# Coloquinte/sleekit

Measured on AMD Instinct MI355X. Metric: Mweights/sec quantized (GPTQ 3-bit, 4096x4096 layer), higher is better.
Workload: dtype f64

## Files before the change

### sleekit_amd/csrc/api.hip

```cpp
#include "mfma32.h"
#include "mfma64.h"

namespace slk {

__global__ __launch_bounds__(256) void k_probe_f64(double *sink, int iters) {
    double4_t c0 = {0, 0, 0, 0}, c1 = c0, c2 = c0, c3 = c0;
    const double a = 1.0 + threadIdx.x * 1e-3, b = 1.0 - threadIdx.x * 1e-3;
    for (int i = 0; i < iters; ++i) {
        c0 = __builtin_amdgcn_mfma_f64_16x16x4f64(a, b, c0, 0, 0, 0);
        c1 = __builtin_amdgcn_mfma_f64_16x16x4f64(b, a, c1, 0, 0, 0);
        c2 = __builtin_amdgcn_mfma_f64_16x16x4f64(a, a, c2, 0, 0, 0);
        c3 = __builtin_amdgcn_mfma_f64_16x16x4f64(b, b, c3, 0, 0, 0);
    }
    const double4_t s = c0 + c1 + c2 + c3;
    if (s[0] + s[1] + s[2] + s[3] == 12345.678) sink[0] = s[0];
}

template <int NACC>
__global__ __launch_bounds__(256) void k_probe_f64_n(double *sink, int iters) {
    double4_t c[NACC];
    double a[NACC], b[NACC];
#pragma unroll
    for (int i = 0; i < NACC; ++i) {
        c[i] = (double4_t){0, 0, 0, 0};
// ... 67 lines not shown
}

using namespace slk;

extern "C" {

int slk_probe_chain(double *out, int iters, int mode, slk_stream_t stream) {
    SLK_REQUIRE(out && iters > 0, "bad arguments");
    hipStream_t s = as_stream(stream);
    SLK_RUN("probe_chain", 0, 0, s, k_probe_chain<<<1, 64, 0, s>>>(out, iters, mode));
    return SLK_OK;
}

size_t slk_workspace_bytes(int R, int n) {
    if (R < 0 || n <= 0) return 0;
    const size_t ld = (size_t)slk_factor_ld(n);
    const size_t rn = (size_t)(R > 0 ? R : 1) * (size_t)n;
    size_t factor = 2 * ld * ld * sizeof(double) + 2 * (ld / 64) * sizeof(int);
    size_t loop = 2 * rn * sizeof(float) + (size_t)n * sizeof(int) + 64 * sizeof(float) + 5 * 256;
    size_t search = rn * sizeof(float) + (size_t)(R + n) * sizeof(float) + (size_t)R * ((n + 127) / 128) * sizeof(float) + 4096;
    size_t error = 6 * (rn + 128 * (size_t)n) + 6 * (size_t)n * n + 4 * (size_t)R * ((n + 127) / 128) * sizeof(float) + 8192;
    size_t prep = 64 * sizeof(float) + (size_t)n * (sizeof(double) + 1);
    search += error;
    size_t m = factor;
    if (loop > m) m = loop;
    if (search > m) m = search;
    if (error > m) m = error;
    if (prep > m) m = prep;
    return m + (1u << 16);
}

size_t slk_workspace_bytes_batch(int batch, int rows_per_layer, int n) {
    if (batch < 1 || batch > 64 || rows_per_layer < 0 || n <= 0 || (long long)batch * rows_per_layer > 0x7fffffffLL) return 0;
    return slk_workspace_bytes(batch * rows_per_layer, n) + (size_t)(batch - 1) * 6 * (size_t)n * n +
           (size_t)batch * n * (sizeof(int) + sizeof(float)) + (size_t)(batch - 1) * 64 * sizeof(float) +
           4096;
}

int slk_probe_mfma_f64(double *sink, int blocks, int iters, slk_stream_t stream) {
    SLK_REQUIRE(sink && blocks > 0 && iters > 0, "bad arguments");
    hipStream_t s = as_stream(stream);
    SLK_RUN("probe_mfma_f64", 4.0 * 2048 * 4 * iters * blocks, 0, s, k_probe_f64<<<blocks, 256, 0, s>>>(sink, iters));
    return SLK_OK;
}

int slk_probe_mfma_f64_acc(double *sink, int blocks, int iters, int nacc, slk_stream_t stream) {
    SLK_REQUIRE(sink && blocks > 0 && iters > 0 && (nacc == 1 || nacc == 2 || nacc == 4 || nacc == 8 || nacc == 16), "bad arguments");
    hipStream_t s = as_stream(stream);
    if (nacc == 1)
        SLK_RUN("probe_mfma_f64", 1.0 * 2048 * 4 * iters * blocks, 0, s, k_probe_f64_n<1><<<blocks, 256, 0, s>>>(sink, iters));
    else if (nacc == 2)
        SLK_RUN("probe_mfma_f64", 2.0 * 2048 * 4 * iters * blocks, 0, s, k_probe_f64_n<2><<<blocks, 256, 0, s>>>(sink, iters));
    else if (nacc == 4)
        SLK_RUN("probe_mfma_f64", 4.0 * 2048 * 4 * iters * blocks, 0, s, k_probe_f64_n<4><<<blocks, 256, 0, s>>>(sink, iters));
    else if (nacc == 8)
        SLK_RUN("probe_mfma_f64", 8.0 * 2048 * 4 * iters * blocks, 0, s, k_probe_f64_n<8><<<blocks, 256, 0, s>>>(sink, iters));
    else
        SLK_RUN("probe_mfma_f64", 16.0 * 2048 * 4 * iters * blocks, 0, s, k_probe_f64_n<16><<<blocks, 256, 0, s>>>(sink, iters));
    return SLK_OK;
}

int slk_probe_mfma_f32(float *sink, int blocks, int iters, slk_stream_t stream) {
    SLK_REQUIRE(sink && blocks > 0 && iters > 0, "bad arguments");
    hipStream_t s = as_stream(stream);
    SLK_RUN("probe_mfma_f32", 4.0 * 4096 * 4 * iters * blocks, 0, s, k_probe_f32<<<blocks, 256, 0, s>>>(sink, iters));
    return SLK_OK;
}

}

#include <atomic>
#include <map>
#include <mutex>
#include <string>
#include <vector>
#include <strings.h>

namespace slk {
namespace {
const char *const kOptNames[OPT_COUNT] = {
    "NO_FAST_LEAF", "NO_DEFER", "NO_WINDOW2", "WIN_DBG", "NO_REGULAR_SEARCH", "NO_FAST_SEARCH_DIV",
    "NO_ERROR_SPLITK", "ERROR_CB", "NO_SYM_ERROR", "NO_BF16_ERROR", "NO_BF16_DMA", "NO_BF16_HESSIAN",
    "ERROR_F32_BELOW", "NO_BF16_ASYM", "NO_SYM_AVERAGE", "NO_WAVE_SEARCH", "LOOKAHEAD", "WINDOW_ROWS", "PANEL_SPLIT", "ROWS_BELOW_WIDE",
    "NO_LOOP_ERROR",
};
std::atomic<int> g_opts[OPT_COUNT];
std::once_flag g_opts_once;
void opts_from_env() {
    for (int i = 0; i < OPT_COUNT; ++i) {
        const std::string name = std::string("SLK_") + kOptNames[i];
        const char *v = getenv(name.c_str());
        int val = 0;
        if (v) {
            val = atoi(v);
            if (val == 0 && v[0] != '0') val = 1;
        }
        g_opts[i].store(val, std::memory_order_relaxed);
    }
}
int opt_index(const char *name) {
    if (!name) return -1;
    if (strncasecmp(name, "SLK_", 4) == 0) name += 4;
    for (int i = 0; i < OPT_COUNT; ++i)
        if (strcasecmp(name, kOptNames[i]) == 0) return i;
    return -1;
}
std::mutex g_lds_mu;
std::map<std::pair<const void *, int>, size_t> g_lds_set;
}

int opt(Opt o) {
    std::call_once(g_opts_once, opts_from_env);
    return g_opts[o].load(std::memory_order_relaxed);
}

namespace {
std::mutex g_helper_mu;
struct HelperRec {
    Helper h;
    int made;
};
std::map<std::pair<int, hipStream_t>, HelperRec> g_helpers;
}

hipError_t helper_for(hipStream_t main, int need, Helper *out) {
    if (need > HELPER_EVENTS) return hipErrorInvalidValue;
    int device = 0;
    hipError_t e = hipGetDevice(&device);
    if (e != hipSuccess) return e;
    std::lock_guard<std::mutex> lock(g_helper_mu);
    auto it = g_helpers.find({device, main});
    if (it == g_helpers.end()) {
        HelperRec r{};
        e = hipStreamCreateWithFlags(&r.h.stream, hipStreamNonBlocking);
        if (e != hipSuccess) return e;
        e = hipStreamCreateWithFlags(&r.h.stream2, hipStreamNonBlocking);
        if (e != hipSuccess) {
            (void)hipStreamDestroy(r.h.stream);
            return e;
        }
        r.h.events = new hipEvent_t[HELPER_EVENTS]();
        r.made = 0;
        it = g_helpers.emplace(std::make_pair(device, main), r).first;
    }
    HelperRec &r = it->second;
    const int had = r.made;
    while (r.made < need) {
        e = hipEventCreateWithFlags(&r.h.events[r.made], hipEventDisableTiming);
        if (e != hipSuccess) {
            while (r.made > had) (void)hipEventDestroy(r.h.events[--r.made]);
            if (had == 0) {
                (void)hipStreamDestroy(r.h.stream);
                (void)hipStreamDestroy(r.h.stream2);
                delete[] r.h.events;
                g_helpers.erase(it);
            }
            return e;
        }
        ++r.made;
    }
    *out = r.h;
    return hipSuccess;
}

static hipError_t release_helpers() {
    std::lock_guard<std::mutex> lock(g_helper_mu);
    hipError_t first = hipSuccess;
// ... 156 lines not shown
```

### sleekit_amd/csrc/common.h

```cpp
#pragma once

#include <hip/hip_runtime.h>
#include <stddef.h>
#include <stdint.h>
#include <stdio.h>

#include "../../include/sleekit_amd.h"

namespace slk {

void set_error(const char *fmt, ...);

#define SLK_REQUIRE(cond, ...)          \
    do {                                \
        if (!(cond)) {                  \
            slk::set_error(__VA_ARGS__); \
            return SLK_E_ARG;           \
        }                               \
    } while (0)

#define SLK_HIP(call)                                                                  \
    do {                                                                               \
        hipError_t e_ = (call);                                                        \
        if (e_ != hipSuccess) {                                                        \
            slk::set_error("%s failed: %s (%s:%d)", #call, hipGetErrorString(e_), __FILE__, __LINE__); \
            return SLK_E_HIP;                                                          \
        }                                                                              \
    } while (0)

#define SLK_LAUNCH_CHECK() SLK_HIP(hipGetLastError())

struct ProfScope {
    int slot;
    hipStream_t stream;
    ProfScope(const char *name, double flops, double bytes, hipStream_t s);
    ~ProfScope();
};

void prof_next_width(long workgroups);

#define SLK_RUN(name, flops, bytes, stream, ...)                 \
    do {                                                         \
        {                                                        \
            slk::ProfScope prof_scope_(name, flops, bytes, stream); \
            __VA_ARGS__;                                         \
        }                                                        \
        SLK_LAUNCH_CHECK();                                      \
    } while (0)

#define SLK_RUN_W(name, flops, bytes, wgs, stream, ...) \
    do {                                                \
        slk::prof_next_width((long)(wgs));              \
        SLK_RUN(name, flops, bytes, stream, __VA_ARGS__); \
    } while (0)

enum Opt {
    OPT_NO_FAST_LEAF,
    OPT_NO_DEFER,
    OPT_NO_WINDOW2,
    OPT_WIN_DBG,
    OPT_NO_REGULAR_SEARCH,
    OPT_NO_FAST_SEARCH_DIV,
    OPT_NO_ERROR_SPLITK,
    OPT_ERROR_CB,
    OPT_NO_SYM_ERROR,
    OPT_NO_BF16_ERROR,
    OPT_NO_BF16_DMA,
    OPT_NO_BF16_HESSIAN,
    OPT_ERROR_F32_BELOW,
    OPT_NO_BF16_ASYM,
    OPT_NO_SYM_AVERAGE,
    OPT_NO_WAVE_SEARCH,
    OPT_LOOKAHEAD,
    OPT_WINDOW_ROWS,
    OPT_PANEL_SPLIT,
    OPT_ROWS_BELOW_WIDE,
    OPT_NO_LOOP_ERROR,
    OPT_COUNT
};
int opt(Opt o);

struct Helper {
    hipStream_t stream;
    hipStream_t stream2;
    hipEvent_t *events;
};
constexpr int HELPER_EVENTS = 512;
hipError_t helper_for(hipStream_t main, int need, Helper *out);

hipError_t lds_opt_in(const void *kernel, size_t bytes);
#define SLK_LDS_OPT_IN(kernel, bytes) SLK_HIP(slk::lds_opt_in(reinterpret_cast<const void *>(kernel), (bytes)))

struct PtrTable {
    const float *p[64];
};

int row_errors_products(const float *W, const float *Q, const float *const *Hs, int batch, int rpl, int n, const int *sym_known,
                        float *row_err, float *G, void *workspace, size_t ws_bytes, slk_stream_t stream);

int loop_error_means(const float *const *Hs, int batch, int n, float *out, hipStream_t s);

static inline hipStream_t as_stream(slk_stream_t s) { return reinterpret_cast<hipStream_t>(s); }

static inline size_t align_up(size_t x, size_t a) { return (x + a - 1) / a * a; }

struct Arena {
    char *base;
    size_t size, used;
    Arena(void *p, size_t bytes) : base(static_cast<char *>(p)), size(bytes), used(0) {}
    template <class T>
    T *take(size_t count) {
        size_t off = align_up(used, 256);
        size_t end = off + count * sizeof(T);
        if (end > size || base == nullptr) return nullptr;
        used = end;
        return reinterpret_cast<T *>(base + off);
    }
};

struct Grid {
    float zero, step, top;
    const float *table;
    int n;
};

static inline Grid make_grid(int levels, double lo, double hi, const float *table = nullptr) {
    Grid g;
    g.zero = (float)lo;
    g.step = (float)((hi - lo) / (double)(levels - 1));
    g.top = (float)(levels - 1);
    g.table = table;
    g.n = levels;
    return g;
}

__device__ __forceinline__ float grid_pos(float x, const Grid g, float shift, float first, float last) {
    float t = (x - g.zero) / g.step;
    t = t + shift;
    t = rintf(t);
    return fminf(fmaxf(t, first), last);
}
__device__ __forceinline__ float grid_val(float t, const Grid g) { return t * g.step + g.zero; }
__device__ __forceinline__ float grid_value(float x, const Grid g) {
    return grid_val(grid_pos(x, g, 0.0f, 0.0f, g.top), g);
}

__device__ __forceinline__ int table_index(float x, const Grid g) {
    const float *lim = g.table + g.n;
    int lo = 0, hi = g.n - 1;
    while (lo < hi) {
        const int mid = (lo + hi) >> 1;
        if (lim[mid] <= x) lo = mid + 1; else hi = mid;
    }
    return lo;
}
__device__ __forceinline__ float cb_value(float x, const Grid g) { return g.table ? g.table[table_index(x, g)] : grid_value(x, g); }
__device__ __forceinline__ int cb_index(float x, const Grid g) {
    return g.table ? table_index(x, g) : (int)grid_pos(x, g, 0.0f, 0.0f, g.top);
}
__device__ __forceinline__ float cb_up(float x, const Grid g) {
// ... 95 lines not shown
```

### sleekit_amd/csrc/factor.hip

```cpp
#include <stdlib.h>

#include "mfma64.h"

namespace slk {

constexpr int PANEL = 64;
constexpr int OUTER_SMALL = 256, OUTER_LARGE = 512;
constexpr int LOOKAHEAD_MIN_TILES = 24;

__device__ long long g_panel_cycles[16];

constexpr int TP = 66;

struct PanelSmem {
    double t[PANEL][TP];
    double x[PANEL][TP];
    double a21[PANEL][TP];
    double lb[PANEL][TP];
    double rdiag[PANEL];
    int early_count;
};

#ifndef NEWTON_STEPS
#define NEWTON_STEPS 2
// ... 775 lines not shown
        const double *p = A + (size_t)(rows0 + (lane >> 4)) * ld + K0 + PANEL * q + 16 * wave + (lane & 15);
        return (double4_t){p[0], p[(size_t)4 * ld], p[(size_t)8 * ld], p[(size_t)12 * ld]};
    };
    TileRegs nx;
    tile_fetch<0>(nx, gx, tile_elem(0, 0), ld);
    double4_t c = load_c(0), cnext = load_c(nb > 1 ? 1 : 0);
    for (int q = 0; q < nb; ++q) {
        for (int s = 0; s <= q; ++s) {
            const bool tri = s == q;
            __syncthreads();
            tile_stash(sm.bt, nx);
            if (tri) blk_store_d(&sm.c[0][16 * wave], lane, c);
            __syncthreads();
            if (!tri) {
                if (s + 1 < q) tile_fetch<0>(nx, ga, tile_elem(q, s + 1), ld);
                else tile_fetch<0>(nx, gx, tile_elem(q, q), ld);
            } else if (q + 1 < nb) {
                tile_fetch<0>(nx, ga, tile_elem(q + 1, 0), ld);
            }
            if (!tri) {
                double4_t acc = {0.0, 0.0, 0.0, 0.0};
#pragma unroll
                for (int kq = 0; kq < 4; ++kq) acc = blk_mma_abt(&sm.own[s][0][16 * kq], &sm.bt[16 * wave][16 * kq], acc, 1.0, lane);
                c = c - acc;
            } else {
                double4_t acc = {0.0, 0.0, 0.0, 0.0};
#pragma unroll
                for (int k = 0; k < 4; ++k)
                    if (k <= wave) acc = blk_mma_abt(&sm.c[0][16 * k], &sm.bt[16 * wave][16 * k], acc, 1.0, lane);
#pragma unroll
                for (int j = 0; j < 4; ++j) A[(size_t)(rows0 + (lane >> 4) + 4 * j) * ld + K0 + PANEL * q + 16 * wave + (lane & 15)] = acc[j];
                blk_store_d(&sm.own[q][0][16 * wave], lane, acc);
                c = cnext;
                if (q + 2 < nb) cnext = load_c(q + 2);
            }
        }
    }
}

__global__ __launch_bounds__(256) void k_syrk_tiles(double *__restrict__ A, int ld, int ti0, int tj0, int ka,
                                                    int kb) {
    __shared__ __attribute__((aligned(16))) Tile64Smem sm;
    A += (size_t)blockIdx.z * ld * ld;
    const int bi = ti0 + blockIdx.y, bj = tj0 + blockIdx.x;
    if (bj > bi) return;
    Acc64 acc;
    acc.zero();
    const int t = threadIdx.x;
    const double *pa = A + ((size_t)bi * TILE + (t >> 2)) * ld + (t & 3) * 8;
    const double *pb = A + ((size_t)bj * TILE + (t >> 2)) * ld + (t & 3) * 8;
    double *pc = A + (size_t)bi * TILE * ld + (size_t)bj * TILE;
    Acc64 old;
    tile64_map(old, [&](int r, int c) { return pc[(size_t)r * ld + c]; });
    tile64_mac<false>(
        acc, sm, ka, kb, [&](int k0, double(&v)[8]) { load8d<true>(pa + k0, v); },
        [&](int k0, double(&v)[8]) { load8d<true>(pb + k0, v); });
    tile64_foreach2(old, acc, [&](int r, int c, double o, double v) { pc[(size_t)r * ld + c] = o - v; });
}

__global__ __launch_bounds__(256) void k_syrk_triangle(double *__restrict__ A, int ld, int t0, int m, int ka, int kb) {
    __shared__ __attribute__((aligned(16))) Tile64Smem sm;
    A += (size_t)blockIdx.z * ld * ld;
    const int total = m * (m + 1) / 2, per_xcd = (total + 7) / 8;
    const int lin = (blockIdx.x & 7) * per_xcd + (blockIdx.x >> 3);
    if (lin >= total) return;
    int row = (int)((sqrtf(8.0f * (float)lin + 1.0f) - 1.0f) * 0.5f);
    while (row * (row + 1) / 2 > lin) --row;
    while ((row + 1) * (row + 2) / 2 <= lin) ++row;
    const int bi = t0 + row, bj = t0 + lin - row * (row + 1) / 2;
    Acc64 acc;
    acc.zero();
    const int t = threadIdx.x;
    const double *pa = A + ((size_t)bi * TILE + (t >> 2)) * ld + (t & 3) * 8;
    const double *pb = A + ((size_t)bj * TILE + (t >> 2)) * ld + (t & 3) * 8;
    tile64_mac<false>(
        acc, sm, ka, kb, [&](int k0, double(&v)[8]) { load8d<true>(pa + k0, v); },
        [&](int k0, double(&v)[8]) { load8d<true>(pb + k0, v); });
    double *pc = A + (size_t)bi * TILE * ld + (size_t)bj * TILE;
    Acc64 old;
    tile64_map(old, [&](int r, int c) { return pc[(size_t)r * ld + c]; });
    tile64_foreach2(old, acc, [&](int r, int c, double o, double v) { pc[(size_t)r * ld + c] = o - v; });
}

template <int STAGE>
__global__ __launch_bounds__(256) void k_trtri_level(const double *__restrict__ L, double *__restrict__ X,
                                                     double *__restrict__ S, int ld, int nt, int s, int node0) {
    __shared__ __attribute__((aligned(16))) Tile64Smem sm;
    L += (size_t)blockIdx.z * ld * ld;
    X += (size_t)blockIdx.z * ld * ld;
    S += (size_t)blockIdx.z * ld * ld;
    const int id = blockIdx.x;
    const int per_node = s * s, node = node0 + id / per_node, in_node = id % per_node;
    const int deep = in_node / s, other = in_node % s;
    const int lo = node * 2 * s, mid = lo + s;
    const int bi = (STAGE == 0) ? mid + other : mid + (s - 1 - deep);
    const int bj = (STAGE == 0) ? lo + deep : lo + other;
    if (bi >= nt) return;
    Acc64 acc;
    acc.zero();
    const int t = threadIdx.x;
    if (STAGE == 0) {
        const double *pa = L + ((size_t)bi * TILE + (t >> 2)) * ld + (t & 3) * 8;
        const double *pb = X + (size_t)(t >> 3) * ld + (size_t)bj * TILE + (t & 7) * 2;
        tile64_mac<true>(
            acc, sm, bj * TILE, mid * TILE, [&](int k0, double(&v)[8]) { load8d<true>(pa + k0, v); },
            [&](int k0, double(&v)[8]) { load8d_cols(pb + (size_t)k0 * ld, v); });
        double *pc = S + (size_t)bi * TILE * ld + (size_t)bj * TILE;
        tile64_foreach(acc, [&](int r, int c, double v) { pc[(size_t)r * ld + c] = v; });
    } else {
        const double *pa = X + ((size_t)bi * TILE + (t >> 2)) * ld + (t & 3) * 8;
        const double *pb = S + (size_t)(t >> 3) * ld + (size_t)bj * TILE + (t & 7) * 2;
        tile64_mac<true>(
            acc, sm, mid * TILE, (bi + 1) * TILE, [&](int k0, double(&v)[8]) { load8d<true>(pa + k0, v); },
            [&](int k0, double(&v)[8]) { load8d_cols(pb + (size_t)k0 * ld, v); });
        double *pc = X + (size_t)bi * TILE * ld + (size_t)bj * TILE;
        tile64_foreach(acc, [&](int r, int c, double v) { pc[(size_t)r * ld + c] = -v; });
    }
}

__global__ __launch_bounds__(256) void k_flip_out(const double *__restrict__ X, int ld, int n,
                                                  double *__restrict__ U) {
    X += (size_t)blockIdx.z * ld * ld;
    U += (size_t)blockIdx.z * n * n;
    for (int i = blockIdx.x; i < n; i += gridDim.x) {
        const double *src = X + (size_t)(n - 1 - i) * ld;
        double *dst = U + (size_t)i * n;
        for (int j = threadIdx.x; j < n; j += blockDim.x) dst[j] = (j >= i) ? src[n - 1 - j] : 0.0;
    }
}

__global__ void k_clear_info(int *info, int *flags, int per_matrix) {
    if (threadIdx.x == 0) info[blockIdx.x] = 0;
    if (flags)
        for (int i = threadIdx.x; i < per_matrix; i += blockDim.x) flags[(size_t)blockIdx.x * per_matrix + i] = 0;
}

}

using namespace slk;

static int chol_inverse_impl(double *A, int batch, int n, double *U, int *info, void *workspace, size_t ws_bytes,
                             slk_stream_t stream, bool want_lookahead) {
    const int ld = slk_factor_ld(n);
    const int nt = ld / TILE;
    const unsigned B = (unsigned)batch;
    const double Bd = (double)batch;
    Arena ws(workspace, ws_bytes);
    double *X = ws.take<double>((size_t)ld * ld * batch);
    double *S = ws.take<double>((size_t)ld * ld * batch);
    int *flags = ws.take<int>((size_t)batch * 2 * nt);
    if (!X || !S || !flags) {
        set_error("workspace too small for %d factorisation(s) of %d x %d", batch, n, n);
        return SLK_E_WS;
    }
    hipStream_t s = as_stream(stream);
    const int OUTER = n >= 4096 ? OUTER_LARGE : OUTER_SMALL;
    SLK_LDS_OPT_IN(k_chol_panel, sizeof(PanelSmem));
    SLK_RUN_W("clear_info", 0, 4, 1, s, k_clear_info<<<B, 64, 0, s>>>(info, flags, 2 * nt));

    Helper helper{};
    const bool lookahead = (want_lookahead || opt(OPT_LOOKAHEAD)) && nt >= LOOKAHEAD_MIN_TILES + OUTER / TILE && nt / (OUTER / TILE) < HELPER_EVENTS / 3;
    if (lookahead) SLK_HIP(helper_for(s, 3 * (nt / (OUTER / TILE) + 1), &helper));
    const int sp = opt(OPT_PANEL_SPLIT);
    const bool chain = (sp == 0 || sp == 3) && slk_chain_addressable(ld);
    const bool split = !chain && !want_lookahead && sp != 2 && (sp == 1 || batch > 1 || n >= 8192);
    if (split) SLK_LDS_OPT_IN(k_panel_below, sizeof(BelowSmem));
    if (chain) {
        SLK_LDS_OPT_IN(k_chol_chain<false>, sizeof(PanelSmem));
        SLK_LDS_OPT_IN(k_chol_chain<true>, sizeof(PanelSmem));
        SLK_LDS_OPT_IN(k_chol_rows_below, sizeof(RowsBelowSmem));
    }
    int inv_done[2][16] = {{0}, {0}};
    auto inverse_nodes = [&](int tiles_done, hipStream_t st) -> int {
        int li = 0;
        for (int lvl = 1; lvl < nt; lvl *= 2, ++li) {
            const int all = (nt + 2 * lvl - 1) / (2 * lvl);
            for (int stage = 0; stage < 2; ++stage) {
                int ready;
                if (tiles_done >= nt) ready = all;
                else if (stage == 0) ready = tiles_done >= lvl ? (tiles_done - lvl) / (2 * lvl) + 1 : 0;
                else ready = tiles_done / (2 * lvl);
                if (ready > all) ready = all;
                const int first = inv_done[stage][li], count = ready - first;
                if (count <= 0) continue;
                inv_done[stage][li] = ready;
                double fl = 0, tiles = 0;
                for (int nd = first; nd < ready; ++nd) {
                    const int lo = nd * 2 * lvl, mid = lo + lvl, hi = lo + 2 * lvl < nt ? lo + 2 * lvl : nt;
                    for (int bi = mid; bi < hi; ++bi)
                        for (int bj = lo; bj < mid; ++bj) {
                            fl += 2.0 * 64 * 64 * 64 * (stage == 0 ? mid - bj : bi + 1 - mid);
                            tiles += 1;
                        }
                }
                if (tiles == 0) continue;
                dim3 grid(count * lvl * lvl, 1, B);
                if (stage == 0)
                    SLK_RUN_W("trtri_stage0", Bd * fl, Bd * (fl / 64 * 8.0 / 2 + tiles * 8.0 * 64 * 64), tiles * batch, st,
                              k_trtri_level<0><<<grid, 256, 0, st>>>(A, X, S, ld, nt, lvl, first));
                else
                    SLK_RUN_W("trtri_stage1", Bd * fl, Bd * (fl / 64 * 8.0 / 2 + tiles * 8.0 * 64 * 64), tiles * batch, st,
                              k_trtri_level<1><<<grid, 256, 0, st>>>(A, X, S, ld, nt, lvl, first));
            }
        }
        return SLK_OK;
    };
    const int EV = chain ? 3 : 2;
    int block = 0, forked = -1;
    int inverse_on_helper = -1;
    for (int K0 = 0; K0 < ld; K0 += OUTER) {
        const int K1 = K0 + OUTER < ld ? K0 + OUTER : ld;
        if (chain) {
            const int nb = (K1 - K0) / PANEL, below_tiles = (ld - K1) / PANEL;
            const double e = 64.0 * nb;
            SLK_RUN_W("chol_chain", Bd * e * e * e / 3.0, Bd * 12.0 * e * e, nb * batch, s,
                      k_chol_chain<false><<<dim3(nb, 1, B), 256, sizeof(PanelSmem), s>>>(A, ld, K0, nb, X, info, flags, opt(OPT_WIN_DBG) & 8));
            if (below_tiles > 0 && forked >= 0) {
                SLK_HIP(hipStreamWaitEvent(s, helper.events[EV * forked + 1], 0));
                forked = -1;
            }
            const int rw = opt(OPT_ROWS_BELOW_WIDE);
            const bool wide = rw == 1 || (rw == 0 && 4 * below_tiles * batch >= 1024);
            if (below_tiles > 0 && wide)
                SLK_RUN_W("chol_rows_below", Bd * 64.0 * below_tiles * e * e, Bd * (16.0 * 64 * below_tiles * e + 4.0 * e * e), below_tiles * batch, s,
                          k_chol_chain<true><<<dim3(below_tiles, 1, B), 256, sizeof(PanelSmem), s>>>(A, ld, K0, nb, X, info, flags, 0));
            else if (below_tiles > 0)
                SLK_RUN_W("chol_rows_below", Bd * 64.0 * below_tiles * e * e, Bd * (16.0 * 64 * below_tiles * e + 4.0 * e * e), 4 * below_tiles * batch, s,
                          k_chol_rows_below<<<dim3(4 * below_tiles, 1, B), 256, sizeof(RowsBelowSmem), s>>>(A, ld, K0, nb, X));
        }
        for (int k0 = K0; k0 < K1 && !chain; k0 += PANEL) {
            const int below = (ld - k0) / PANEL;
            const int kprev = k0 > K0 ? k0 - PANEL : -1;
            const int rest_cols = kprev >= 0 ? (K1 - k0) / PANEL - 1 : 0;
            int rest = 0;
            for (int c = 0; c < rest_cols; ++c) rest += nt - (k0 / TILE + 1 + c);
            const double prologue = kprev >= 0 ? (double)below * 2.0 * 64 * 64 * 64 + (double)below * 2.0 * 64 * 64 * 64 : 0.0;
            if (split) {
                const double pro1 = kprev >= 0 ? 2.0 * 64 * 64 * 64 : 0.0;
                SLK_RUN_W("chol_panel", Bd * (2.0 / 3.0 * 64 * 64 * 64 + pro1), Bd * 16.0 * 64 * 64, batch, s,
                          k_chol_panel<<<dim3(1, 1, B), 256, sizeof(PanelSmem), s>>>(A, ld, k0, kprev, 1, 0, X, info, opt(OPT_WIN_DBG) & 8));
                if (below - 1 + rest > 0) {
                    const int per_wg = 2;
                    const int nbw = (below - 1 + per_wg - 1) / per_wg;
                    SLK_RUN_W("chol_panel_below",
                              Bd * ((double)(below - 1) * 64 * 64 * 64 + (kprev >= 0 ? (double)(below - 1) * 2.0 * 64 * 64 * 64 : 0.0) +
                                    (double)rest * 2.0 * 64 * 64 * PANEL),
                              Bd * (24.0 * (below - 1) * 64 * 64 + (double)rest * 16.0 * 64 * 64), (nbw + rest) * batch, s,
                              k_panel_below<<<dim3(nbw + rest, 1, B), 256, sizeof(BelowSmem), s>>>(A, ld, k0, kprev, nbw, rest_cols, X, below - 1,
                                                                                                  per_wg));
                }
            } else {
                SLK_RUN_W("chol_panel",
                          Bd * (2.0 / 3.0 * 64 * 64 * 64 + (double)(below - 1) * 64 * 64 * 64 + prologue + (double)rest * 2.0 * 64 * 64 * PANEL),
                          Bd * (16.0 * below * 64 * 64 + (double)rest * 16.0 * 64 * 64), (below + rest) * batch, s,
                          k_chol_panel<<<dim3(below + rest, 1, B), 256, sizeof(PanelSmem), s>>>(A, ld, k0, kprev, below, rest_cols, X, info,
                                                                                                opt(OPT_WIN_DBG) & 8));
            }
        }
        const int t0 = K1 / TILE;
        if (nt > t0) {
            const int m = nt - t0, total = m * (m + 1) / 2;
            const double tiles = total;
            const int ahead = OUTER / TILE;
            if (lookahead && chain && m >= LOOKAHEAD_MIN_TILES) {
                SLK_HIP(hipEventRecord(helper.events[EV * block], s));
                const int nbn = ahead < m ? ahead : m, td = nbn * (nbn + 1) / 2;
                SLK_RUN_W("chol_syrk_ahead", Bd * td * 2.0 * 64 * 64 * (K1 - K0), Bd * (16.0 * nbn * 64 * (K1 - K0) + td * 16.0 * 64 * 64), td * batch, s,
                          k_syrk_tiles<<<dim3(nbn, nbn, B), 256, 0, s>>>(A, ld, t0, t0, K0, K1));
                SLK_HIP(hipStreamWaitEvent(helper.stream, helper.events[EV * block], 0));
                const int m2 = m - nbn, total2 = m2 * (m2 + 1) / 2;
                if (m2 > 0) {
                    SLK_RUN_W("chol_syrk_outer", Bd * (double)nbn * m2 * 2.0 * 64 * 64 * (K1 - K0), Bd * (8.0 * (ld - K1) * (K1 - K0) + (double)nbn * m2 * 16.0 * 64 * 64),
                              (double)nbn * m2 * batch, helper.stream,
                              k_syrk_tiles<<<dim3(nbn, m2, B), 256, 0, helper.stream>>>(A, ld, t0 + nbn, t0, K0, K1));
                    SLK_RUN_W("chol_syrk_outer", Bd * total2 * 2.0 * 64 * 64 * (K1 - K0), Bd * (8.0 * (ld - K1) * (K1 - K0) + total2 * 16.0 * 64 * 64),
                              (double)total2 * batch, helper.stream,
                              k_syrk_triangle<<<dim3(8 * ((total2 + 7) / 8), 1, B), 256, 0, helper.stream>>>(A, ld, t0 + nbn, m2, K0, K1));
                }
                SLK_HIP(hipEventRecord(helper.events[EV * block + 1], helper.stream));
                forked = block;
                SLK_HIP(hipStreamWaitEvent(helper.stream2, helper.events[EV * block], 0));
                {
                    const int rc = inverse_nodes(t0, helper.stream2);
                    if (rc != SLK_OK) return rc;
                }
                SLK_HIP(hipEventRecord(helper.events[EV * block + 2], helper.stream2));
                inverse_on_helper = block;
            } else if (lookahead && m >= LOOKAHEAD_MIN_TILES) {
                if (block > 0) SLK_HIP(hipStreamWaitEvent(s, helper.events[2 * (block - 1) + 1], 0));
                SLK_HIP(hipEventRecord(helper.events[2 * block], s));
                const double ta = (double)ahead * m - 6;
                SLK_RUN_W("chol_syrk_ahead", Bd * ta * 2.0 * 64 * 64 * (K1 - K0), Bd * (8.0 * (ld - K1) * (K1 - K0) + ta * 16.0 * 64 * 64),
                          ta * batch, s, k_syrk_tiles<<<dim3(ahead, m, B), 256, 0, s>>>(A, ld, t0, t0, K0, K1));
                SLK_HIP(hipStreamWaitEvent(helper.stream, helper.events[2 * block], 0));
                const int m2 = m - ahead, total2 = m2 * (m2 + 1) / 2;
                SLK_RUN_W("chol_syrk_outer", Bd * total2 * 2.0 * 64 * 64 * (K1 - K0), Bd * (8.0 * (ld - K1) * (K1 - K0) + total2 * 16.0 * 64 * 64),
                          (double)total2 * batch, helper.stream,
                          k_syrk_triangle<<<dim3(8 * ((total2 + 7) / 8), 1, B), 256, 0, helper.stream>>>(A, ld, t0 + ahead, m2, K0, K1));
                SLK_HIP(hipEventRecord(helper.events[2 * block + 1], helper.stream));
                forked = block;
            } else {
                if (forked >= 0) {
                    SLK_HIP(hipStreamWaitEvent(s, helper.events[EV * forked + 1], 0));
                    forked = -1;
                }
                if (lookahead && chain) {
                    SLK_HIP(hipEventRecord(helper.events[EV * block], s));
                    SLK_HIP(hipStreamWaitEvent(helper.stream2, helper.events[EV * block], 0));
                    const int rc = inverse_nodes(t0, helper.stream2);
                    if (rc != SLK_OK) return rc;
                    SLK_HIP(hipEventRecord(helper.events[EV * block + 2], helper.stream2));
                    inverse_on_helper = block;
                }
                SLK_RUN_W("chol_syrk_outer", Bd * tiles * 2.0 * 64 * 64 * (K1 - K0), Bd * (8.0 * (ld - K1) * (K1 - K0) + tiles * 16.0 * 64 * 64),
                          tiles * batch, s, k_syrk_triangle<<<dim3(8 * ((total + 7) / 8), 1, B), 256, 0, s>>>(A, ld, t0, m, K0, K1));
            }
        }
        ++block;
    }
    if (forked >= 0) SLK_HIP(hipStreamWaitEvent(s, helper.events[EV * forked + 1], 0));
    if (inverse_on_helper >= 0) SLK_HIP(hipStreamWaitEvent(s, helper.events[EV * inverse_on_helper + 2], 0));
    {
        const int rc = inverse_nodes(nt, s);
        if (rc != SLK_OK) return rc;
    }
    SLK_RUN("flip_out", 0, Bd * 12.0 * n * n, s, k_flip_out<<<dim3(n < 2048 ? n : 2048, 1, B), 256, 0, s>>>(X, ld, n, U));
    return SLK_OK;
}

extern "C" int slk_chol_inverse_upper(double *A, int n, double *U, int *info, void *workspace,
                                      size_t ws_bytes, slk_stream_t stream) {
    SLK_REQUIRE(A && U && info && n > 0, "bad arguments");
    return chol_inverse_impl(A, 1, n, U, info, workspace, ws_bytes, stream, false);
}

extern "C" int slk_chol_inverse_upper_lookahead(double *A, int n, double *U, int *info, void *workspace,
                                                size_t ws_bytes, slk_stream_t stream) {
    SLK_REQUIRE(A && U && info && n > 0, "bad arguments");
    return chol_inverse_impl(A, 1, n, U, info, workspace, ws_bytes, stream, true);
}

extern "C" int slk_chol_inverse_upper_batch(double *A, int batch, int n, double *U, int *info, void *workspace,
                                            size_t ws_bytes, slk_stream_t stream) {
    SLK_REQUIRE(A && U && info && n > 0, "bad arguments");
    SLK_REQUIRE(batch >= 1 && batch <= 64, "batch must be 1..64");
    return chol_inverse_impl(A, batch, n, U, info, workspace, ws_bytes, stream, false);
}

extern "C" int slk_probe_panel_cycles(long long *host_out, int reset) {
    SLK_REQUIRE(host_out, "null pointer");
    SLK_HIP(hipDeviceSynchronize());
    SLK_HIP(hipMemcpyFromSymbol(host_out, HIP_SYMBOL(g_panel_cycles), sizeof(long long) * 16));
    if (reset) {
        long long zero[16] = {0};
        SLK_HIP(hipMemcpyToSymbol(HIP_SYMBOL(g_panel_cycles), zero, sizeof(zero)));
    }
    return SLK_OK;
}

extern "C" size_t slk_factor_workspace_bytes_batch(int batch, int n) {
    if (batch < 1 || batch > 64 || n <= 0) return 0;
    const size_t ld = (size_t)slk_factor_ld(n);
    return 2 * ld * ld * sizeof(double) * batch + (size_t)batch * (64 * sizeof(float) + (size_t)n * (sizeof(double) + sizeof(int))) +
           (size_t)batch * 2 * (ld / 64) * sizeof(int) + (1u << 16);
}
```

### sleekit_amd/csrc/mfma64.h

```cpp
#pragma once

#include <type_traits>

#include "common.h"

namespace slk {

typedef double double4_t __attribute__((ext_vector_type(4)));
typedef double double2_t __attribute__((ext_vector_type(2)));
typedef float float4v_t __attribute__((ext_vector_type(4)));

constexpr int TILE = 64;
constexpr int KSTEP = 32;
constexpr int PITCH_RK = 34;
constexpr int PITCH_KC = 80;

struct Tile64Smem {
    double a[TILE * PITCH_RK];
    double b[KSTEP * PITCH_KC];
};

constexpr int PITCH_AF = 36;
struct Tile64SmemAf {
    float a[TILE * PITCH_AF];
    double b[KSTEP * PITCH_KC];
};

struct Acc64 {
    double4_t c[2][2];
    __device__ __forceinline__ void zero() {
#pragma unroll
        for (int i = 0; i < 2; ++i)
#pragma unroll
            for (int j = 0; j < 2; ++j) c[i][j] = (double4_t){0.0, 0.0, 0.0, 0.0};
    }
};

template <bool VEC>
__device__ __forceinline__ void load8d(const double *p, double (&v)[8]) {
    if (VEC) {
#pragma unroll
        for (int h = 0; h < 4; ++h) {
            const double2_t x = *reinterpret_cast<const double2_t *>(p + 2 * h);
            v[2 * h] = x[0];
            v[2 * h + 1] = x[1];
        }
    } else {
#pragma unroll
        for (int e = 0; e < 8; ++e) v[e] = p[e];
    }
}

__device__ __forceinline__ void load8d_cols(const double *p, double (&v)[8]) {
#pragma unroll
    for (int h = 0; h < 4; ++h) {
        const double2_t x = *reinterpret_cast<const double2_t *>(p + 16 * h);
        v[2 * h] = x[0];
        v[2 * h + 1] = x[1];
    }
}
__device__ __forceinline__ void load8d_cols_guarded(const double *row, int c2, int last, bool ok, double (&v)[8]) {
#pragma unroll
    for (int e = 0; e < 8; ++e) {
        const int col = 16 * (e >> 1) + c2 + (e & 1);
        v[e] = row[min(col, max(last, 0))] * ((ok && col <= last) ? 1.0 : 0.0);
    }
}

__device__ __forceinline__ void load8d_guarded(const double *p, int last, bool ok, double (&v)[8]) {
#pragma unroll
    for (int e = 0; e < 8; ++e) v[e] = p[min(e, max(last, 0))] * ((ok && e <= last) ? 1.0 : 0.0);
}

template <bool VEC>
__device__ __forceinline__ void load8f_as_d(const float *p, double (&v)[8]) {
    if (VEC) {
        const float4v_t lo = *reinterpret_cast<const float4v_t *>(p), hi = *reinterpret_cast<const float4v_t *>(p + 4);
#pragma unroll
        for (int e = 0; e < 4; ++e) {
            v[e] = (double)lo[e];
            v[4 + e] = (double)hi[e];
        }
    } else {
#pragma unroll
        for (int e = 0; e < 8; ++e) v[e] = (double)p[e];
    }
}
template <bool VEC>
__device__ __forceinline__ void load8f(const float *p, float (&v)[8]) {
    if (VEC) {
        const float4v_t lo = *reinterpret_cast<const float4v_t *>(p), hi = *reinterpret_cast<const float4v_t *>(p + 4);
#pragma unroll
        for (int e = 0; e < 4; ++e) {
            v[e] = lo[e];
            v[4 + e] = hi[e];
        }
    } else {
#pragma unroll
        for (int e = 0; e < 8; ++e) v[e] = p[e];
    }
}
__device__ __forceinline__ void load8f_guarded(const float *p, int last, bool ok, float (&v)[8]) {
#pragma unroll
    for (int e = 0; e < 8; ++e) v[e] = p[min(e, max(last, 0))] * ((ok && e <= last) ? 1.0f : 0.0f);
}
__device__ __forceinline__ void load8f_as_d_guarded(const float *p, int last, bool ok, double (&v)[8]) {
#pragma unroll
    for (int e = 0; e < 8; ++e) v[e] = (double)p[min(e, max(last, 0))] * ((ok && e <= last) ? 1.0 : 0.0);
}

template <bool B_C_FAST, class TA = double, class SM, class LA, class LB>
__device__ __forceinline__ void tile64_mac(Acc64 &acc, SM &sm, int k_begin, int k_end, LA la, LB lb) {
    constexpr bool AF = std::is_same<SM, Tile64SmemAf>::value;
    static_assert(!AF || (std::is_same<TA, float>::value && B_C_FAST), "the float32 A image is for float32 A and column-contiguous B");
    using TL = typename std::conditional<AF, float, double>::type;
    constexpr int PITCH_A = AF ? PITCH_AF : PITCH_RK;
    const int t = threadIdx.x;
    const int lane = t & 63, wave = t >> 6;
    const int wr = wave >> 1, wc = wave & 1;
    TA ra[8];
    double rb[8];
    TL *a_dst = sm.a + (t >> 2) * PITCH_A + (t & 3) * 8;
    double *b_dst = B_C_FAST ? sm.b + (t >> 3) * PITCH_KC + (t & 7) * 2 : sm.b + (t >> 2) * PITCH_RK + (t & 3) * 8;
    constexpr int B_PIECE = B_C_FAST ? 16 : 2;

    auto stash = [&]() {
        if constexpr (AF) {
#pragma unroll
            for (int h = 0; h < 2; ++h)
                *reinterpret_cast<float4v_t *>(a_dst + 4 * h) = (float4v_t){(float)ra[4 * h], (float)ra[4 * h + 1], (float)ra[4 * h + 2], (float)ra[4 * h + 3]};
        }
#pragma unroll
        for (int h = 0; h < 4; ++h) {
            if constexpr (!AF) *reinterpret_cast<double2_t *>(a_dst + 2 * h) = (double2_t){(double)ra[2 * h], (double)ra[2 * h + 1]};
            *reinterpret_cast<double2_t *>(b_dst + B_PIECE * h) = (double2_t){rb[2 * h], rb[2 * h + 1]};
        }
    };

    if (k_begin >= k_end) return;
    la(k_begin, ra);
    lb(k_begin, rb);
// ... 92 lines not shown
```

Measured before the change: 5583.

## Write triangular inverse directly into flipped output, dropping final flip pass

When n equals ld, the blocked triangular inverse now writes stage-1 results straight into the flipped U layout, zeroes the mirrored tiles, and flips diagonal tiles with a small per-tile kernel. Later stages read already-finished off-diagonal blocks back from U through reversed loads. The full-matrix flip_out kernel is skipped in that case. This removes one whole n×n read/write pass but adds scalar reversed loads and extra stores inside the trtri kernels.

```diff
diff --git a/sleekit_amd/csrc/api.hip b/sleekit_amd/csrc/api.hip
--- a/sleekit_amd/csrc/api.hip
+++ b/sleekit_amd/csrc/api.hip
@@ -173,7 +173,7 @@
     "NO_FAST_LEAF", "NO_DEFER", "NO_WINDOW2", "WIN_DBG", "NO_REGULAR_SEARCH", "NO_FAST_SEARCH_DIV",
     "NO_ERROR_SPLITK", "ERROR_CB", "NO_SYM_ERROR", "NO_BF16_ERROR", "NO_BF16_DMA", "NO_BF16_HESSIAN",
     "ERROR_F32_BELOW", "NO_BF16_ASYM", "NO_SYM_AVERAGE", "NO_WAVE_SEARCH", "LOOKAHEAD", "WINDOW_ROWS", "PANEL_SPLIT", "ROWS_BELOW_WIDE",
-    "NO_LOOP_ERROR",
+    "NO_LOOP_ERROR", "FLIP_PASS",
 };
 std::atomic<int> g_opts[OPT_COUNT];
 std::once_flag g_opts_once;
diff --git a/sleekit_amd/csrc/common.h b/sleekit_amd/csrc/common.h
--- a/sleekit_amd/csrc/common.h
+++ b/sleekit_amd/csrc/common.h
@@ -76,6 +76,7 @@
     OPT_PANEL_SPLIT,
     OPT_ROWS_BELOW_WIDE,
     OPT_NO_LOOP_ERROR,
+    OPT_FLIP_PASS,
     OPT_COUNT
 };
 int opt(Opt o);
diff --git a/sleekit_amd/csrc/factor.hip b/sleekit_amd/csrc/factor.hip
--- a/sleekit_amd/csrc/factor.hip
+++ b/sleekit_amd/csrc/factor.hip
@@ -881,13 +881,14 @@
     tile64_foreach2(old, acc, [&](int r, int c, double o, double v) { pc[(size_t)r * ld + c] = o - v; });
 }
 
-template <int STAGE>
+template <int STAGE, bool TO_U>
 __global__ __launch_bounds__(256) void k_trtri_level(const double *__restrict__ L, double *__restrict__ X,
-                                                     double *__restrict__ S, int ld, int nt, int s, int node0) {
+                                                     double *__restrict__ S, double *U, int ld, int nt, int s, int node0) {
     __shared__ __attribute__((aligned(16))) Tile64Smem sm;
     L += (size_t)blockIdx.z * ld * ld;
     X += (size_t)blockIdx.z * ld * ld;
     S += (size_t)blockIdx.z * ld * ld;
+    if (TO_U) U += (size_t)blockIdx.z * ld * ld;
     const int id = blockIdx.x;
     const int per_node = s * s, node = node0 + id / per_node, in_node = id % per_node;
     const int deep = in_node / s, other = in_node % s;
@@ -898,22 +899,60 @@
     Acc64 acc;
     acc.zero();
     const int t = threadIdx.x;
+    const size_t last = (size_t)ld - 1;
+    int one = 1;
+    if (TO_U) asm volatile("" : "+v"(one));
     if (STAGE == 0) {
         const double *pa = L + ((size_t)bi * TILE + (t >> 2)) * ld + (t & 3) * 8;
         const double *pb = X + (size_t)(t >> 3) * ld + (size_t)bj * TILE + (t & 7) * 2;
+        const double *pu = !TO_U ? nullptr : U + (last - (t >> 3)) * ld + (last - (size_t)bj * TILE - (t & 7) * 2);
+        const int diag_end = (bj + 1) * TILE;
         tile64_mac<true>(
             acc, sm, bj * TILE, mid * TILE, [&](int k0, double(&v)[8]) { load8d<true>(pa + k0, v); },
-            [&](int k0, double(&v)[8]) { load8d_cols(pb + (size_t)k0 * ld, v); });
+            [&](int k0, double(&v)[8]) {
+                if (!TO_U || k0 < diag_end) load8d_cols(pb + (size_t)k0 * ld, v);
+                else load8d_cols_rev(pu - (size_t)k0 * ld, pu - (size_t)k0 * ld - one, v);
+            });
         double *pc = S + (size_t)bi * TILE * ld + (size_t)bj * TILE;
         tile64_foreach(acc, [&](int r, int c, double v) { pc[(size_t)r * ld + c] = v; });
     } else {
         const double *pa = X + ((size_t)bi * TILE + (t >> 2)) * ld + (t & 3) * 8;
         const double *pb = S + (size_t)(t >> 3) * ld + (size_t)bj * TILE + (t & 7) * 2;
+        const double *pu = !TO_U ? nullptr : U + (last - (size_t)bi * TILE - (t >> 2)) * ld + (last - (t & 3) * 8);
+        const int diag_begin = bi * TILE;
         tile64_mac<true>(
-            acc, sm, mid * TILE, (bi + 1) * TILE, [&](int k0, double(&v)[8]) { load8d<true>(pa + k0, v); },
+            acc, sm, mid * TILE, (bi + 1) * TILE,
+            [&](int k0, double(&v)[8]) {
+                if (!TO_U || k0 >= diag_begin) load8d<true>(pa + k0, v);
+                else load8d_rev(pu - k0, pu - k0 - one, v);
+            },
             [&](int k0, double(&v)[8]) { load8d_cols(pb + (size_t)k0 * ld, v); });
-        double *pc = X + (size_t)bi * TILE * ld + (size_t)bj * TILE;
-        tile64_foreach(acc, [&](int r, int c, double v) { pc[(size_t)r * ld + c] = -v; });
+        if (TO_U) {
+            double *pc = U + (last - (size_t)bi * TILE) * ld + (last - (size_t)bj * TILE);
+            tile64_foreach(acc, [&](int r, int c, double v) { pc[-(ptrdiff_t)((size_t)r * ld + c)] = -v; });
+            double *pz = U + ((size_t)(nt - 1 - bj) * TILE + (t >> 5)) * ld + (size_t)(nt - 1 - bi) * TILE + (t & 31) * 2;
+#pragma unroll
+            for (int i = 0; i < 8; ++i) *reinterpret_cast<double2_t *>(pz + (size_t)(8 * i) * ld) = (double2_t){0.0, 0.0};
+        } else {
+            double *pc = X + (size_t)bi * TILE * ld + (size_t)bj * TILE;
+            tile64_foreach(acc, [&](int r, int c, double v) { pc[(size_t)r * ld + c] = -v; });
+        }
+    }
+}
+
+__global__ __launch_bounds__(256) void k_flip_diag(const double *__restrict__ X, int n, int t0, double *__restrict__ U) {
+    X += (size_t)blockIdx.z * n * n;
+    U += (size_t)blockIdx.z * n * n;
+    const int d = t0 + blockIdx.x, t = threadIdx.x;
+    const double *src = X + (size_t)d * TILE * n + (size_t)d * TILE;
+    const size_t ud = (size_t)n - TILE - (size_t)d * TILE;
+    double *dst = U + ud * n + ud;
+    const int j = (t & 31) * 2;
+#pragma unroll
+    for (int k = 0; k < 8; ++k) {
+        const int i = (t >> 5) + 8 * k;
+        const double2_t x = *reinterpret_cast<const double2_t *>(src + (size_t)(63 - i) * n + 62 - j);
+        *reinterpret_cast<double2_t *>(dst + (size_t)i * n + j) = (double2_t){j >= i ? x[1] : 0.0, j + 1 >= i ? x[0] : 0.0};
     }
 }
 
@@ -969,8 +1008,17 @@
         SLK_LDS_OPT_IN(k_chol_chain<true>, sizeof(PanelSmem));
         SLK_LDS_OPT_IN(k_chol_rows_below, sizeof(RowsBelowSmem));
     }
+    const bool direct = n == ld && !opt(OPT_FLIP_PASS);
+    int diag_done = 0;
     int inv_done[2][16] = {{0}, {0}};
     auto inverse_nodes = [&](int tiles_done, hipStream_t st) -> int {
+        if (direct) {
+            const int upto = tiles_done < nt ? tiles_done : nt;
+            if (upto > diag_done)
+                SLK_RUN_W("flip_diag", 0, Bd * 12.0 * 64 * 64 * (upto - diag_done), (upto - diag_done) * batch, st,
+                          k_flip_diag<<<dim3(upto - diag_done, 1, B), 256, 0, st>>>(X, n, diag_done, U));
+            if (upto > diag_done) diag_done = upto;
+        }
         int li = 0;
         for (int lvl = 1; lvl < nt; lvl *= 2, ++li) {
             const int all = (nt + 2 * lvl - 1) / (2 * lvl);
@@ -994,12 +1042,15 @@
                 }
                 if (tiles == 0) continue;
                 dim3 grid(count * lvl * lvl, 1, B);
-                if (stage == 0)
-                    SLK_RUN_W("trtri_stage0", Bd * fl, Bd * (fl / 64 * 8.0 / 2 + tiles * 8.0 * 64 * 64), tiles * batch, st,
-                              k_trtri_level<0><<<grid, 256, 0, st>>>(A, X, S, ld, nt, lvl, first));
+                const double bytes = Bd * (fl / 64 * 8.0 / 2 + tiles * 8.0 * 64 * 64 * (direct && stage == 1 ? 2 : 1));
+                if (stage == 0 && direct)
+                    SLK_RUN_W("trtri_stage0", Bd * fl, bytes, tiles * batch, st, k_trtri_level<0, true><<<grid, 256, 0, st>>>(A, X, S, U, ld, nt, lvl, first));
+                else if (stage == 0)
+                    SLK_RUN_W("trtri_stage0", Bd * fl, bytes, tiles * batch, st, k_trtri_level<0, false><<<grid, 256, 0, st>>>(A, X, S, nullptr, ld, nt, lvl, first));
+                else if (direct)
+                    SLK_RUN_W("trtri_stage1", Bd * fl, bytes, tiles * batch, st, k_trtri_level<1, true><<<grid, 256, 0, st>>>(A, X, S, U, ld, nt, lvl, first));
                 else
-                    SLK_RUN_W("trtri_stage1", Bd * fl, Bd * (fl / 64 * 8.0 / 2 + tiles * 8.0 * 64 * 64), tiles * batch, st,
-                              k_trtri_level<1><<<grid, 256, 0, st>>>(A, X, S, ld, nt, lvl, first));
+                    SLK_RUN_W("trtri_stage1", Bd * fl, bytes, tiles * batch, st, k_trtri_level<1, false><<<grid, 256, 0, st>>>(A, X, S, nullptr, ld, nt, lvl, first));
             }
         }
         return SLK_OK;
@@ -1123,7 +1174,7 @@
         const int rc = inverse_nodes(nt, s);
         if (rc != SLK_OK) return rc;
     }
-    SLK_RUN("flip_out", 0, Bd * 12.0 * n * n, s, k_flip_out<<<dim3(n < 2048 ? n : 2048, 1, B), 256, 0, s>>>(X, ld, n, U));
+    if (!direct) SLK_RUN("flip_out", 0, Bd * 12.0 * n * n, s, k_flip_out<<<dim3(n < 2048 ? n : 2048, 1, B), 256, 0, s>>>(X, ld, n, U));
     return SLK_OK;
 }
 
diff --git a/sleekit_amd/csrc/mfma64.h b/sleekit_amd/csrc/mfma64.h
--- a/sleekit_amd/csrc/mfma64.h
+++ b/sleekit_amd/csrc/mfma64.h
@@ -57,6 +57,20 @@
         const double2_t x = *reinterpret_cast<const double2_t *>(p + 16 * h);
         v[2 * h] = x[0];
         v[2 * h + 1] = x[1];
+    }
+}
+__device__ __forceinline__ void load8d_rev(const double *p, const double *q, double (&v)[8]) {
+#pragma unroll
+    for (int h = 0; h < 4; ++h) {
+        v[2 * h] = p[-2 * h];
+        v[2 * h + 1] = q[-2 * h];
+    }
+}
+__device__ __forceinline__ void load8d_cols_rev(const double *p, const double *q, double (&v)[8]) {
+#pragma unroll
+    for (int h = 0; h < 4; ++h) {
+        v[2 * h] = p[-16 * h];
+        v[2 * h + 1] = q[-16 * h];
     }
 }
 __device__ __forceinline__ void load8d_cols_guarded(const double *row, int c2, int last, bool ok, double (&v)[8]) {
```

Result: no change. 5577 (-0.1%).
